# miloknowles/adaptive-stereo-icra-2021

Hardware: AMD Instinct MI355X
Metric: stereo pairs/sec (fwd+adapt-step), KITTI 1242x375 D=192 (higher is better)
Workload: dtype f32; 1 GPU; KITTI-2015 1242x375, maxdisp 192, k=4 (Dc=12, 24x78 cost volume), forward + one online-adapt step (train-mode BN, monodepth loss, clip 1.0, Adam lr 5e-5); pairs_per_gpu=4, global_batch=4, parallelism=dp1 (per-replica BatchNorm statistics, one flat RCCL gradient all-reduce), kernels=all hand-written HIP (no MIOpen/rocBLAS on the path)

## Files before the change

adaptive-stereo-icra-2021_amd/adaptive_stereo/_native.py:

```python
import ctypes
import os

import torch

_HERE = os.path.dirname(os.path.abspath(__file__))
LIB_PATH = os.path.join(_HERE, "libadaptive_stereo_hip.so")
BUILD_HINT = "build it with: make -C %s" % os.path.join(os.path.dirname(_HERE), "csrc")

c_int, c_float, c_i64, c_vp = ctypes.c_int, ctypes.c_float, ctypes.c_int64, ctypes.c_void_p


class Pcl(ctypes.Structure):
  _fields_ = [(n, ctypes.c_int32) for n in ("B", "D", "H", "W", "pd", "ph", "pw")]

  def numel(self):
    return self.B * (self.D + 2 * self.pd) * (self.H + 2 * self.ph) * (self.W + 2 * self.pw) * 32

  def voxels(self):
    return self.B * self.D * self.H * self.W

  def key(self):
    return (self.B, self.D, self.H, self.W, self.pd, self.ph, self.pw)


# ... 54 lines not shown
  "as_conv32to1_bnsums_ok": (c_int, [_P(Pcl), _P(ConvShape)]),
  "as_conv32to1_bnsums_parts": (c_int, [_P(Pcl)]),
  "as_conv32to1_dgrad_bnsums": (c_int, [c_vp, _P(Pcl), _P(ConvShape), c_vp, c_vp, c_vp, c_vp, c_vp, c_vp, c_float, c_vp, c_vp]),
  "as_wgrad_defer": (c_int, [c_int]),
  "as_wgrad_defer_pending": (c_int, []),
  "as_wgrad_defer_flush": (c_int, [c_vp]),
  "as_conv32_act_ok": (c_int, [_P(Pcl), _P(Pcl), _P(ConvShape)]),
  "as_conv32_act_parts": (c_int, []),
  "as_conv32_act_fwd": (c_int, [c_vp, c_vp, c_vp, c_vp, c_vp, _P(Pcl), c_vp, c_vp, c_float, c_vp, _P(Pcl), _P(ConvShape), c_vp, c_vp,
                                c_vp, c_vp]),
  "as_conv32_wino_ok": (c_int, [_P(Pcl), _P(Pcl), _P(ConvShape)]),
  "as_conv32_wino_parts": (c_int, []),
  "as_conv32_wino_pack_weights": (c_int, [c_vp, c_vp, c_int, c_vp]),
  "as_conv32_wino_fwd": (c_int, [c_vp, c_vp, c_vp, c_vp, c_vp, _P(Pcl), c_vp, c_vp, c_float, c_vp, _P(Pcl), _P(ConvShape), c_vp, c_vp,
                                 c_vp, c_vp]),
  "as_conv32_wino_eval": (c_int, [c_vp, _P(Pcl), _P(ConvShape), c_vp, c_vp, c_vp, c_vp, c_float, c_int, c_vp, c_vp]),
  "as_conv32_wino_bwd_data": (c_int, [c_vp, c_vp, _P(Pcl), _P(ConvShape), c_vp, c_vp, c_vp, c_vp, c_vp, c_float, c_vp, c_vp, c_vp, c_vp,
                                      c_vp, c_vp, c_vp, c_vp]),
  "as_conv32_wino_bwd_filter": (c_int, [c_vp, c_vp, _P(Pcl), _P(ConvShape), c_vp, c_vp, c_int, c_vp, c_vp]),
  "as_conv32_wino_bwd_parts": (c_int, []),
  "as_conv32_wino_bwd_workspace": (c_i64, []),
  "as_conv32_wino_bwd_generation": (c_int, [c_int]),
  "as_conv32_wino_bwd": (c_int, [c_vp, _P(Pcl), c_vp, c_vp, _P(Pcl), _P(ConvShape), c_vp, c_vp, c_vp, c_vp, c_vp, c_float, c_vp,
                                 c_vp, c_vp, c_vp, c_vp, c_vp, c_vp, c_vp, c_int, c_vp, c_vp, c_vp]),
  "as_conv32_wino_bwd_fused_parts": (c_int, []),
  "as_conv32_wino_bwd_fused_workspace": (c_i64, []),
  "as_conv32_wino_bwd_fused": (c_int, [c_vp, _P(Pcl), c_vp, c_vp, _P(Pcl), _P(ConvShape), c_vp, c_vp, c_vp, c_vp, c_vp, c_float, c_vp,
                                       c_vp, c_vp, c_vp, c_vp, c_vp, c_vp, c_int, c_vp, c_vp, c_vp]),
  "as_conv3d_wgrad_lds_assignment": (c_int, [c_int, c_int, c_int, c_vp, c_vp, c_vp]),
  "as_conv32_s2_enable": (c_int, [c_int]),
  "as_conv4_s2_enable": (c_int, [c_int]),
  "as_refine_out_ok": (c_int, [_P(Pcl)]),
  "as_refine_out_fwd": (c_int, [c_vp, c_vp, c_vp, c_vp, c_float, c_vp, _P(Pcl), c_vp, c_vp, c_vp, c_int, c_vp, c_vp]),
  "as_conv32_bwd_fused_ok": (c_int, [_P(Pcl), _P(Pcl), _P(ConvShape)]),
  "as_conv32_bwd_fused_parts": (c_int, []),
  "as_conv32_bwd_fused_workspace": (c_i64, []),
  "as_conv32_bwd_fused": (c_int, [c_vp, _P(Pcl), c_vp, c_vp, _P(Pcl), _P(ConvShape), c_vp, c_vp, c_vp, c_vp, c_vp, c_float, c_vp, c_vp,
                                  c_vp, c_vp, c_vp, c_vp, c_vp, c_int, c_vp, c_vp, c_vp]),
  "as_conv32_bnbwd_parts": (c_int, [_P(Pcl), _P(Pcl), _P(ConvShape)]),
  "as_conv32_fwd_bnbwd": (c_int, [c_vp, _P(Pcl), c_vp, c_vp, _P(Pcl), _P(ConvShape), c_vp, c_vp, c_vp, c_vp, c_vp, c_float,
                                  c_vp, c_vp]),
  "as_agg3d_ok": (c_int, [_P(Pcl)]),
  "as_agg3d_parts": (c_int, [_P(Pcl)]),
  "as_agg3d_fwd": (c_int, [c_vp, _P(Pcl), c_vp, c_vp, c_vp, c_vp, _P(BnMerge), c_vp, c_vp, c_int, c_vp, c_vp, c_float, c_vp, c_vp,
                           c_vp, c_vp]),
  "as_trunk_parts": (c_int, [_P(Pcl), c_int]),
  "as_trunk_fwd": (c_int, [c_vp, c_vp, _P(TrunkBn), c_vp, _P(Pcl), c_int, c_vp, c_vp, c_float, c_vp, c_vp, c_vp, c_vp, c_vp]),
  "as_trunk_finish_fwd": (c_int, [c_vp, _P(Pcl), c_vp, c_vp, c_int, c_int, _P(c_vp), _P(c_vp), c_float, c_vp]),
  "as_trunk_begin_bwd": (c_int, [c_vp, c_vp, c_int, _P(Pcl), c_vp, c_vp]),
  "as_trunk_bwd_workspace": (c_i64, [_P(Pcl), c_int]),
  "as_trunk_bwd": (c_int, [c_vp, c_vp, c_vp, c_vp, c_int, c_vp, c_vp, c_vp, c_vp, c_vp, c_vp, c_vp, c_vp, _P(Pcl), c_int, c_float,
                           c_vp, c_vp, c_int, c_vp, c_vp]),
  "as_trunk_finish_bwd": (c_int, [c_vp, c_int, c_int, _P(c_vp), _P(c_vp), c_int, c_vp]),
  "as_agg_tail_ok": (c_int, [_P(Pcl)]),
  "as_agg_tail_fwd": (c_int, [c_vp, _P(Pcl), c_vp, c_vp, _P(BnMerge), c_vp, c_vp, c_vp, c_float, c_vp, c_vp, c_vp, c_vp, c_vp]),
  "as_conv3d_out_fwd": (c_int, [c_vp, _P(Pcl), c_vp, c_vp, c_vp, c_vp]),
  "as_conv3d_out_bwd_workspace": (c_i64, [_P(Pcl)]),
  "as_conv3d_out_bwd": (c_int, [c_vp, c_vp, _P(Pcl), c_vp, c_vp, c_vp, c_vp, c_int, c_vp, c_vp]),
  "as_conv32to1_fwd": (c_int, [c_vp, _P(Pcl), _P(ConvShape), c_vp, c_vp, c_vp, c_int, c_vp, c_vp]),
  "as_conv32to1_bwd_workspace": (c_i64, [_P(Pcl), _P(ConvShape)]),
  "as_conv32to1_bwd": (c_int, [c_vp, c_vp, _P(Pcl), _P(ConvShape), c_vp, c_vp, c_vp, c_vp, c_int, c_vp, c_vp]),
  "as_pcl4_numel": (c_i64, [_P(Pcl)]),
  "as_pack_in4": (c_int, [c_vp, c_vp, c_int, c_vp, _P(Pcl), c_vp]),
  "as_conv4_pack_weights": (c_int, [c_vp, c_int, c_vp, _P(ConvShape), c_vp]),
  "as_conv4_wgrad_bnapply_ok": (c_int, [_P(Pcl), _P(Pcl), _P(ConvShape)]),
  "as_conv4_wgrad_bnapply_proj": (c_int, [c_vp, _P(Pcl), c_vp, c_vp, _P(Pcl), _P(ConvShape), c_int, c_vp, c_vp, c_vp, c_vp, c_float,
# ... 112 lines not shown
```

adaptive-stereo-icra-2021_amd/adaptive_stereo/hip_ops.py:

```python
import os
import torch

from . import _native as nat
from ._native import Pcl, ConvShape, call, ptr, stream, f32c

LEAKY_SLOPE = 0.2
BN_EPS = 1e-5
BN_MOMENTUM = 0.1

CONV3D_333 = ConvShape(3, 3, 3, 1, 1, 1, 1, 1)

_DIRECT_GRADS = True


def set_direct_grad_accumulation(flag: bool):
  global _DIRECT_GRADS
  _DIRECT_GRADS = bool(flag)


def grad_sinks(params):
  if not (_DIRECT_GRADS and torch.is_grad_enabled()):
    return None
  out = []
  for p in params:
# ... 107 lines not shown
  if not _DeferredReduce.on:
    return
  lib = nat.load()
  lib.as_wgrad_defer(0)
  _DeferredReduce.on = False
  call("as_wgrad_defer_flush", stream())
  _DeferredReduce.keep = []


_TAIL_BNSUMS = True
_HEAD_PROJ = True
_FWD_ACT = True
_WINOGRAD = os.environ.get("AS_DIAG_DIRECT_FORM") != "1"


def set_tail_bnsums(enabled):
  global _TAIL_BNSUMS
  prev, _TAIL_BNSUMS = _TAIL_BNSUMS, bool(enabled)
  return prev


def set_head_proj(enabled):
  global _HEAD_PROJ
  prev, _HEAD_PROJ = _HEAD_PROJ, bool(enabled)
  return prev


_REFINE_OUT = True


def set_refine_out(enabled):
  global _REFINE_OUT
  prev, _REFINE_OUT = _REFINE_OUT, bool(enabled)
  return prev


def set_head_staged(enabled):
  lib = nat.load()
  prev = lib.as_conv32_s2_enable(2) == 1 and lib.as_conv4_s2_enable(2) == 1
  lib.as_conv32_s2_enable(1 if enabled else 0)
  lib.as_conv4_s2_enable(1 if enabled else 0)
  return prev


def set_fwd_act(enabled):
  global _FWD_ACT
  prev, _FWD_ACT = _FWD_ACT, bool(enabled)
  return prev


_WINOGRAD_BWD = True
_WINOGRAD_BWD_ONE_LAUNCH = True


def set_winograd_bwd_one_launch(flag: bool):
  global _WINOGRAD_BWD_ONE_LAUNCH
  prev, _WINOGRAD_BWD_ONE_LAUNCH = _WINOGRAD_BWD_ONE_LAUNCH, bool(flag)
  return prev


def set_winograd(enabled, backward=None):
  global _WINOGRAD, _WINOGRAD_BWD
  prev, _WINOGRAD = _WINOGRAD, bool(enabled)
  _WINOGRAD_BWD = bool(enabled if backward is None else backward)
  return prev

# ... 1098 lines not shown
        a0 = POOL.get(g, dev)
        call("as_conv4_fwd", ptr(in4), g4, ptr(wp4), ptr(b0), ptr(a0), g, s33, 1, ptr(st0.scale), ptr(st0.shift),
             LEAKY_SLOPE, None, None, None, stream())
    if not need_bwd and z0 is not None:
      POOL.put(z0, g); z0 = None

    xs, zs, sts = [a0], [], []
    tail_fused = None
    if fused_act:
      xs = []
      z_prev, st_prev = z0, st0
      for l, dil in enumerate(REFINE_DILATIONS):
        wl, bl, gamma, beta = params[4 + 4 * l:8 + 4 * l]
        rm, rv = bn_buffers[1 + l]
        a_prev, z, st = block_forward_act(z_prev, xs[-1] if xs else None, st_prev, g, conv_shape_2d(dil), wl, bl, gamma, beta,
                                          rm, rv)
        xs.append(a_prev); zs.append(z); sts.append(st)
        z_prev, st_prev = z, st
      if _REFINE_OUT and lib.as_refine_out_ok(g) == 1:
        tail_fused = (z_prev, xs[-1], st_prev)
      else:
        xs.append(bn_act(z_prev, st_prev, g, residual=xs[-1]))
    else:
      for l, dil in enumerate(REFINE_DILATIONS):
        wl, bl, gamma, beta = params[4 + 4 * l:8 + 4 * l]
        rm, rv = bn_buffers[1 + l]
        z, a, st = block_forward(xs[-1], g, conv_shape_2d(dil), wl, bl, gamma, beta, rm, rv, train, True, need_bwd)
        zs.append(z); sts.append(st); xs.append(a)
        if not need_bwd:
          POOL.put(xs[-2], g)

    w_out, b_out = params[28], params[29]
    out = torch.empty(B, 1, H, W, dtype=torch.float32, device=dev)
    if tail_fused is not None:
      z6, a5, st6 = tail_fused
      a6 = POOL.get(g, dev)
      call("as_refine_out_fwd", ptr(z6), ptr(a5), ptr(st6.scale), ptr(st6.shift), LEAKY_SLOPE, ptr(a6), g, ptr(w_out), ptr(b_out),
           ptr(up), 1, ptr(out), stream())
      xs.append(a6)
    elif _REFINE_OUT and lib.as_refine_out_ok(g) == 1:
      call("as_refine_out_fwd", ptr(xs[-1]), None, None, None, LEAKY_SLOPE, None, g, ptr(w_out), ptr(b_out), ptr(up), 1, ptr(out),
           stream())
    else:
      call("as_conv32to1_fwd", ptr(xs[-1]), g, s33, ptr(w_out), ptr(b_out), ptr(up), 1, ptr(out), stream())

    if need_bwd:
      ctx.g, ctx.g4, ctx.train = g, g4, bool(train)
      ctx.sinks = sinks
      ctx.dims = (B, h, w, H, W, float(gain))
      ctx.in4, ctx.z0, ctx.st0 = in4, z0, st0
      ctx.xs, ctx.zs, ctx.sts = xs, zs, sts
      ctx.save_for_backward(out, *params)
    else:
      POOL.put(xs[-1], g); POOL.put(in4, g4, channels=4)
    return out

  @staticmethod
  def backward(ctx, g_out):
    out, *params = ctx.saved_tensors
    g, g4 = ctx.g, ctx.g4
    B, h, w, H, W, gain = ctx.dims
    dev = out.device
    lib = nat.load()
    s33 = conv_shape_2d(1)
    xs, zs, sts = ctx.xs, ctx.zs, ctx.sts
    grads = [None] * 30

    g_out = f32c(g_out)
    g_pre = torch.empty_like(out)
    call("as_relu_bwd", ptr(g_out), ptr(out), out.numel(), ptr(g_pre), stream())
    w_out = params[28]
    sinks = ctx.sinks
    g_a = POOL.get(g, dev)
    ws = _empty(lib.as_conv32to1_bwd_workspace(g, s33), dev)
    sums = None
    if _sink(sinks, 28) is not None and _sink(sinks, 29) is not None:
      if _TAIL_BNSUMS and ctx.train and _BN_SYNC is None and lib.as_conv32to1_bnsums_ok(g, s33) == 1:
        nws = _empty(lib.as_bn_bwd_workspace(g), dev)
        ev = fork_beside(lambda: call("as_conv32to1_bwd", ptr(g_pre), ptr(xs[6]), g, s33, ptr(w_out), None, ptr(sinks[28]),
                                      ptr(sinks[29]), 1, ptr(ws), stream()))
        call("as_conv32to1_dgrad_bnsums", ptr(g_pre), g, s33, ptr(w_out), ptr(g_a), ptr(zs[5]), ptr(sts[5].scale),
             ptr(sts[5].shift), ptr(sts[5].mean), LEAKY_SLOPE, ptr(nws), stream())
        join_beside(ev)
        sums = BnBwdSums(nws, lib.as_conv32to1_bnsums_parts(g))
      else:
        call("as_conv32to1_bwd", ptr(g_pre), ptr(xs[6]), g, s33, ptr(w_out), ptr(g_a), ptr(sinks[28]), ptr(sinks[29]), 1,
             ptr(ws), stream())
    else:
      g_wout, g_bout = torch.empty_like(w_out), _empty(1, dev)
      call("as_conv32to1_bwd", ptr(g_pre), ptr(xs[6]), g, s33, ptr(w_out), ptr(g_a), ptr(g_wout), ptr(g_bout), 0,
           ptr(ws), stream())
      grads[28], grads[29] = g_wout, g_bout

    for l in range(5, -1, -1):
      wl, bl, gamma, beta = params[4 + 4 * l:8 + 4 * l]
      next_bn = (zs[l - 1], sts[l - 1]) if l > 0 else (ctx.z0, ctx.st0)
      g_x, dW, db, g_gamma, g_beta, sums = block_backward(g_a, xs[l], zs[l], sts[l], wl, gamma, g,
                                                          conv_shape_2d(REFINE_DILATIONS[l]), ctx.train, True, True,
                                                          sinks[4 + 4 * l:8 + 4 * l] if sinks is not None else None,
                                                          sums, next_bn)
      grads[4 + 4 * l:8 + 4 * l] = [dW, db, g_gamma, g_beta]
      POOL.put(g_a, g); POOL.put(zs[l], g); POOL.put(xs[l + 1], g)
      g_a = g_x

    w0, b0, gamma0, beta0 = params[0:4]
    ws4 = _empty(lib.as_conv4_wgrad_workspace(g, s33), dev)
    all_sinks = all(_sink(sinks, i) is not None for i in range(4))
    if all_sinks and lib.as_conv4_wgrad_bnapply_ok(g4, g, s33) == 1:
      bws = sums.workspace if sums is not None else _empty(lib.as_bn_bwd_workspace(g), dev)
      st0 = ctx.st0
      bn_bwd_coefs(g_a, ctx.z0, st0, gamma0, g, ctx.train, sinks[2], sinks[3], True, bws, sums)
      coef = bws[lib.as_bn_bwd_coef_offset():]
      if _HEAD_PROJ and ctx.needs_input_grad[0] and not ctx.needs_input_grad[1]:
        w_proj = pack_special(w0, PACK_MIRROR_TAP, 9, 288,
                              lambda w_, o_: call("as_mirror_taps_ch0", ptr(w_), 4, ptr(o_), None, stream()))
        h_proj = _empty(B * 9 * H * W, dev)
        call("as_conv4_wgrad_bnapply_proj", ptr(ctx.in4), g4, ptr(g_a), ptr(ctx.z0), g, s33, 4, ptr(st0.scale), ptr(st0.shift),
             ptr(st0.mean), ptr(coef), LEAKY_SLOPE, ptr(w_proj), ptr(h_proj), ptr(sinks[0]), ptr(sinks[1]), 1, ptr(ws4),
             stream())
        g_z0 = None
      else:
        h_proj = None
        g_z0 = POOL.get(g, dev)
        call("as_conv4_wgrad_bnapply", ptr(ctx.in4), g4, ptr(g_a), ptr(ctx.z0), g, s33, 4, ptr(st0.scale), ptr(st0.shift),
             ptr(st0.mean), ptr(coef), LEAKY_SLOPE, ptr(g_z0), ptr(sinks[0]), ptr(sinks[1]), 1, ptr(ws4), stream())
      dW0 = db0 = g_gamma0 = g_beta0 = None
    else:
      h_proj = None
      g_z0, g_gamma0, g_beta0 = bn_act_bwd(g_a, ctx.z0, ctx.st0, gamma0, g, ctx.train, _sink(sinks, 2), _sink(sinks, 3), sums)
      if _sink(sinks, 0) is not None and _sink(sinks, 1) is not None:
        call("as_conv4_wgrad", ptr(ctx.in4), g4, ptr(g_z0), g, s33, 4, ptr(sinks[0]), ptr(sinks[1]), 1, ptr(ws4), stream())
        dW0 = db0 = None
      else:
        dW0 = torch.empty_like(w0); db0 = _empty(32, dev)
        call("as_conv4_wgrad", ptr(ctx.in4), g4, ptr(g_z0), g, s33, 4, ptr(dW0), ptr(db0), 0, ptr(ws4), stream())
# ... 219 lines not shown
```

adaptive-stereo-icra-2021_amd/csrc/refine_out.hip:

```cpp
#include "as_common.h"

#define RO_COLS 126
#ifndef RO_ROWS_ACT
#define RO_ROWS_ACT 32
#endif
#ifndef RO_ROWS_PLAIN
#define RO_ROWS_PLAIN 12
#endif
#define RO_PW 132

struct RefineOutArgs {
  const float* x;
  const float* skip;
  const float* scale;
  const float* shift;
  float* a_out;
  const float* w;
  const float* bias;
  const float* add_src;
  float* out;
  PclDev g;
  int nseg, nstrips, relu;
  float slope;
};

template <bool ACT>
__global__ __launch_bounds__(256) void refine_out_kernel(RefineOutArgs p) {
  __shared__ __attribute__((aligned(16))) char xrow[128 * 128];
  __shared__ float P[3][9][RO_PW];
  const int t = threadIdx.x, lane = t & 63, wave = t >> 6;
  const int h = lane >> 5, li = lane & 31;
  const int H = p.g.H, W = p.g.W;
  int blk = blockIdx.x;
  const int seg = blk % p.nseg; blk /= p.nseg;
  const int strip = blk % p.nstrips;
  const int b = blk / p.nstrips;
  const int x0 = seg * RO_COLS;
  constexpr int ROWS = ACT ? RO_ROWS_ACT : RO_ROWS_PLAIN;
  const int ya = strip * ROWS, yb = min(H, ya + ROWS);

  float Bw[16];
#pragma unroll
  for (int i = 0; i < 16; ++i) Bw[i] = li < 9 ? p.w[(16 * h + i) * 9 + li] : 0.f;
  const float bias = p.bias ? p.bias[0] : 0.f;

  const int cq = t & 7, v0 = t >> 3;
  const int lds_w = v0 * 128 + ((cq ^ ((v0 >> 1) & 7)) << 4);
  f32x4 sc = {0.f, 0.f, 0.f, 0.f}, sh = {0.f, 0.f, 0.f, 0.f};
  if (ACT) { sc = *reinterpret_cast<const f32x4*>(p.scale + cq * 4); sh = *reinterpret_cast<const f32x4*>(p.shift + cq * 4); }
  unsigned colmask = 0u, ownmask = 0u;
#pragma unroll
  for (int k = 0; k < 4; ++k) {
    const int v = v0 + 32 * k, xx = x0 - 1 + v;
    colmask |= ((xx >= 0 && xx < W) ? 1u : 0u) << k;
    ownmask |= ((v >= 1 && v <= RO_COLS && xx < W) ? 1u : 0u) << k;
  }
  const long row0 = (((long)b * p.g.Hp + p.g.ph) * p.g.Wp + (x0 - 1 + p.g.pw)) * 32 + t * 4;
  auto fetch = [&](int yi, f32x4 (&rz)[4], f32x4 (&rs)[4]) {
    const long off = row0 + (long)min(max(yi, 0), H - 1) * p.g.Wp * 32;
#pragma unroll
    for (int k = 0; k < 4; ++k) {
      rz[k] = *reinterpret_cast<const f32x4*>(p.x + off + k * 1024);
      if (ACT && p.skip) rs[k] = *reinterpret_cast<const f32x4*>(p.skip + off + k * 1024);
    }
  };
  const int mv = 32 * wave + li;
  const char* a_rd = xrow + mv * 128;
  const int a_sw = (mv >> 1) & 7;

  f32x4 rz[4], rs[4];
#pragma unroll
  for (int k = 0; k < 4; ++k) rs[k] = (f32x4){0.f, 0.f, 0.f, 0.f};
  fetch(ya - 1, rz, rs);
  for (int yi = ya - 1; yi <= yb; ++yi) {
    const bool row_in = yi >= 0 && yi < H;
    const bool row_own = yi >= ya && yi < yb;
#pragma unroll
    for (int k = 0; k < 4; ++k) {
      f32x4 y = rz[k];
      if (ACT) {
        y = y * sc + sh;
        y.x = y.x > 0.f ? y.x : y.x * p.slope; y.y = y.y > 0.f ? y.y : y.y * p.slope;
        y.z = y.z > 0.f ? y.z : y.z * p.slope; y.w = y.w > 0.f ? y.w : y.w * p.slope;
        if (p.skip) y += rs[k];
      }
      if (!row_in || !((colmask >> k) & 1u)) y = (f32x4){0.f, 0.f, 0.f, 0.f};
      *reinterpret_cast<f32x4*>(xrow + lds_w + k * 4096) = y;
      if (ACT && row_own && ((ownmask >> k) & 1u))
        *reinterpret_cast<f32x4*>(p.a_out + row0 + (long)yi * p.g.Wp * 32 + k * 1024) = y;
    }
    if (yi < yb) fetch(yi + 1, rz, rs);
    __syncthreads();
    f32x16 acc;
    {
      f32x4 xa[4];
#pragma unroll
      for (int q = 0; q < 4; ++q) xa[q] = *reinterpret_cast<const f32x4*>(a_rd + (((4 * h + q) ^ a_sw) << 4));
      const f32x16 zero = {0.f, 0.f, 0.f, 0.f, 0.f, 0.f, 0.f, 0.f, 0.f, 0.f, 0.f, 0.f, 0.f, 0.f, 0.f, 0.f};
      acc = __builtin_amdgcn_mfma_f32_32x32x2f32(xa[0].x, Bw[0], zero, 0, 0, 0);
      acc = __builtin_amdgcn_mfma_f32_32x32x2f32(xa[0].y, Bw[1], acc, 0, 0, 0);
      acc = __builtin_amdgcn_mfma_f32_32x32x2f32(xa[0].z, Bw[2], acc, 0, 0, 0);
      acc = __builtin_amdgcn_mfma_f32_32x32x2f32(xa[0].w, Bw[3], acc, 0, 0, 0);
#pragma unroll
      for (int q = 1; q < 4; ++q) {
        acc = __builtin_amdgcn_mfma_f32_32x32x2f32(xa[q].x, Bw[4 * q + 0], acc, 0, 0, 0);
        acc = __builtin_amdgcn_mfma_f32_32x32x2f32(xa[q].y, Bw[4 * q + 1], acc, 0, 0, 0);
        acc = __builtin_amdgcn_mfma_f32_32x32x2f32(xa[q].z, Bw[4 * q + 2], acc, 0, 0, 0);
        acc = __builtin_amdgcn_mfma_f32_32x32x2f32(xa[q].w, Bw[4 * q + 3], acc, 0, 0, 0);
      }
    }
    if (li < 9) {
      float* pr = &P[(yi + 1) % 3][li][32 * wave + 4 * h];
#pragma unroll
      for (int r = 0; r < 16; ++r) pr[(r & 3) + 8 * (r >> 2)] = acc[r];
    }
    __syncthreads();
    const int yo = yi - 1;
    if (yo >= ya && t < RO_COLS && x0 + t < W) {
      float s = bias;
#pragma unroll
      for (int ky = 0; ky < 3; ++ky) {
        const float (*pr)[RO_PW] = P[(yo + ky) % 3];
#pragma unroll
        for (int kx = 0; kx < 3; ++kx) s += pr[ky * 3 + kx][t + kx];
      }
      const long o = ((long)b * H + yo) * W + x0 + t;
      if (p.add_src) s += p.add_src[o];
      if (p.relu) s = s > 0.f ? s : 0.f;
      p.out[o] = s;
    }
  }
}

extern "C" int as_refine_out_ok(const as_pcl* g) {
  if (!as_pcl_ok(g)) return 0;
  return g->D == 1 && g->pd == 0 && g->ph >= 1 && g->pw >= 1 && (long)g->ph * (g->W + 2 * g->pw) >= 128 ? 1 : 0;
}

extern "C" int as_refine_out_fwd(const float* x, const float* skip, const float* scale, const float* shift, float slope,
                                 float* a_out, const as_pcl* g, const float* w, const float* bias, const float* add_src,
                                 int relu, float* out, void* stream) {
  AS_CHECK_ARG(as_refine_out_ok(g) == 1, "as_refine_out_fwd: geometry not supported (as_refine_out_ok() == 0)");
  AS_CHECK_ARG(x && w && out, "as_refine_out_fwd: null pointer");
  AS_CHECK_ARG((scale == nullptr) == (shift == nullptr) && (scale == nullptr) == (a_out == nullptr),
               "as_refine_out_fwd: scale, shift and a_out come together (the fused BatchNorm + LeakyReLU) or not at all");
  AS_CHECK_ARG(scale != nullptr || skip == nullptr, "as_refine_out_fwd: a skip connection needs the fused activation");
  AS_CHECK_ARG(a_out == nullptr || (a_out != x && a_out != skip), "as_refine_out_fwd: a_out must not alias an input");
  AS_CHECK_ARG(scale == nullptr || (slope > 0.f && slope < 1.f), "as_refine_out_fwd: slope must lie in (0, 1)");
  RefineOutArgs a;
  a.x = x; a.skip = skip; a.scale = scale; a.shift = shift; a.a_out = a_out; a.w = w; a.bias = bias; a.add_src = add_src;
  a.out = out; a.g = as_make_dev(g); a.relu = relu; a.slope = slope;
  a.nseg = as_div_up(g->W, RO_COLS); a.nstrips = as_div_up(g->H, scale ? RO_ROWS_ACT : RO_ROWS_PLAIN);
  const int grid = g->B * a.nseg * a.nstrips;
  if (scale) hipLaunchKernelGGL(refine_out_kernel<true>, dim3(grid), dim3(256), 0, (hipStream_t)stream, a);
  else hipLaunchKernelGGL(refine_out_kernel<false>, dim3(grid), dim3(256), 0, (hipStream_t)stream, a);
  AS_CHECK_LAUNCH("as_refine_out_fwd");
  return AS_OK;
}
```

adaptive-stereo-icra-2021_amd/csrc/softargmax.hip:

```cpp
#include "as_common.h"

struct OutGeom {
  int kd, kh, kw, pad_d, pad_h, pad_w, dil, ntaps;
  int tap_off[27];
};

struct OutConvArgs {
  const float* a;
  const float* w;
  const float* bias;
  const float* add_src;
  float* out;
  int relu;
  PclDev g;
  long M;
  OutGeom k;
};

__global__ __launch_bounds__(256) void conv32to1_fwd_kernel(OutConvArgs p) {
  __shared__ float sw[27 * 32];
  const int NT = p.k.ntaps;
  for (int i = threadIdx.x; i < NT * 32; i += 256) {
    const int t = i >> 5, c = i & 31;
    sw[i] = p.w[c * NT + t];
// ... 349 lines not shown
        const int vx = f >> 3;
        const f32x4 av = it == 0 ? a4[0][k4] : a4[1][k4];
        if (c4 == 0) gsum += sgc[1][vx + 1];
#pragma unroll
        for (int ky = 0; ky < 3; ++ky)
#pragma unroll
          for (int kx = 0; kx < 3; ++kx) acc[ky * 3 + kx] += sgc[2 - ky][vx + 2 - kx] * av;
      }
    }
  }
  float* out = p.partial + (long)blockIdx.x * (9 * 32 + 1);
#pragma unroll
  for (int tp = 0; tp < 9; ++tp) {
    __syncthreads();
    red[vl][c4 * 4 + 0] = acc[tp].x; red[vl][c4 * 4 + 1] = acc[tp].y;
    red[vl][c4 * 4 + 2] = acc[tp].z; red[vl][c4 * 4 + 3] = acc[tp].w;
    __syncthreads();
    if (threadIdx.x < 32) {
      float s = 0.f;
      for (int j = 0; j < 32; ++j) s += red[j][threadIdx.x];
      out[tp * 32 + threadIdx.x] = s;
    }
  }
  __syncthreads();
  if (c4 == 0) red[vl][0] = gsum;
  __syncthreads();
  if (threadIdx.x == 0) {
    float s = 0.f;
    for (int j = 0; j < 32; ++j) s += red[j][0];
    out[9 * 32] = s;
  }
}

static bool thin2d_applicable(const as_pcl* g, const as_conv_shape* s) {
  return g->D == 1 && s->kd == 1 && s->kh == 3 && s->kw == 3 && s->dil == 1 && s->stride == 1 && s->pad_h == 1 &&
         s->pad_w == 1 && g->ph >= 1 && g->pw >= 1 && (long)g->B * g->H * ((g->W + 127) / 128) < (1L << 31);
}

__global__ __launch_bounds__(256) void softargmax_fwd_kernel(const float* __restrict__ logits, int B, int D, long HW,
                                                              float* __restrict__ pred, int32_t* __restrict__ argmax,
                                                              float* __restrict__ fcs) {
  const long i = (long)blockIdx.x * 256 + threadIdx.x;
  if (i >= (long)B * HW) return;
  const long b = i / HW, pix = i % HW;
  const float* l = logits + b * D * HW + pix;
  float m1 = -INFINITY, m2 = -INFINITY, sum = 0.f;
  int am = 0;
  for (int d = 0; d < D; ++d) {
    const float v = l[d * HW];
    sum += v;
    if (v > m1) { m2 = m1; m1 = v; am = d; }
    else if (v > m2) { m2 = v; }
  }
  float se = 0.f;
  for (int d = 0; d < D; ++d) se += expf(l[d * HW] - m1);
  float acc = 0.f;
  for (int d = 0; d < D; ++d) acc += (expf(l[d * HW] - m1) / se) * (float)d;
  pred[i] = acc;
  if (argmax) argmax[i] = am;
  if (fcs) fcs[i] = (D > 2) ? m1 - (sum - m1 - m2) / (float)(D - 2) : 0.f;
}

__global__ __launch_bounds__(256) void softargmax_bwd_kernel(const float* __restrict__ logits, const float* __restrict__ g_pred,
                                                              const float* __restrict__ g_in, int B, int D, long HW,
                                                              float* __restrict__ g_logits) {
  const long i = (long)blockIdx.x * 256 + threadIdx.x;
// ... 116 lines not shown
    hipLaunchKernelGGL(conv32to1_wgrad_reduce_kernel, dim3(as_div_up(p.k.ntaps * 32 + 1, 4)), dim3(256), 0, st,
                       workspace, (int)nb, p.k.ntaps, g_w, g_bias, accumulate);
    AS_CHECK_LAUNCH("as_conv32to1_bwd(reduce)");
  }
  return AS_OK;
}

#define THIN_BNSUMS_BLOCKS 1024
extern "C" int as_conv32to1_bnsums_ok(const as_pcl* g, const as_conv_shape* s) {
  if (!g || !s || !as_pcl_ok(g)) return AS_ERR_ARG;
  return thin2d_applicable(g, s) ? 1 : 0;
}
extern "C" int as_conv32to1_bnsums_parts(const as_pcl* g) {
  if (!g || !as_pcl_ok(g)) return AS_ERR_ARG;
  const long nch = (long)g->B * g->H * ((g->W + 127) / 128);
  return (int)(nch < THIN_BNSUMS_BLOCKS ? nch : THIN_BNSUMS_BLOCKS);
}
extern "C" int as_conv32to1_dgrad_bnsums(const float* g_out, const as_pcl* g, const as_conv_shape* s, const float* w, float* g_a,
                                         const float* bn_z, const float* bn_scale, const float* bn_shift, const float* bn_mean,
                                         float slope, float* bn_workspace, void* stream) {
  AS_CHECK_ARG(g && s && as_pcl_ok(g) && thin2d_applicable(g, s), "as_conv32to1_dgrad_bnsums: configuration not supported");
  AS_CHECK_ARG(g_out && w && g_a && bn_z && bn_scale && bn_shift && bn_mean && bn_workspace, "as_conv32to1_dgrad_bnsums: null pointer");
  AS_CHECK_ARG(((uintptr_t)bn_workspace & 7) == 0, "as_conv32to1_dgrad_bnsums: workspace must be 8-byte aligned");
  Thin2dBwdArgs q;
  q.g_out = g_out; q.a = nullptr; q.w = w; q.g_a = g_a; q.partial = nullptr; q.g = as_make_dev(g);
  q.chunks_per_row = (g->W + 127) / 128; q.nchunks = g->B * g->H * q.chunks_per_row;
  q.bn_z = bn_z; q.bn_scale = bn_scale; q.bn_shift = bn_shift; q.bn_mean = bn_mean; q.slope = slope;
  q.bn_partial = reinterpret_cast<double*>(bn_workspace);
  hipLaunchKernelGGL(conv32to1_2d_dgrad_kernel<true>, dim3(as_conv32to1_bnsums_parts(g)), dim3(256), 0, (hipStream_t)stream, q);
  AS_CHECK_LAUNCH("as_conv32to1_dgrad_bnsums");
  return AS_OK;
}

static const as_conv_shape k333 = {3, 3, 3, 1, 1, 1, 1, 1};

extern "C" int as_conv3d_out_fwd(const float* a, const as_pcl* g, const float* w, const float* bias,
                                 float* logits, void* stream) {
  as_prof_mark(AS_PROF_OUTCONV_FWD, (hipStream_t)stream, 1, 0.0);
  const int e = as_conv32to1_fwd(a, g, &k333, w, bias, nullptr, 0, logits, stream);
  if (e == AS_OK && g) as_prof_mark(AS_PROF_OUTCONV_FWD, (hipStream_t)stream, 0, (128.0 + 4.0) * (double)g->B * g->D * g->H * g->W);
  return e;
}

extern "C" int64_t as_conv3d_out_bwd_workspace(const as_pcl* g) { return as_conv32to1_bwd_workspace(g, &k333); }

extern "C" int as_conv3d_out_bwd(const float* g_logits, const float* a, const as_pcl* g, const float* w,
                                 float* g_a, float* g_w, float* g_bias, int accumulate, float* workspace, void* stream) {
  AS_CHECK_ARG(g_a && g_w, "as_conv3d_out_bwd: null pointer");
  as_prof_mark(AS_PROF_OUTCONV_BWD, (hipStream_t)stream, 1, 0.0);
  const int e = as_conv32to1_bwd(g_logits, a, g, &k333, w, g_a, g_w, g_bias, accumulate, workspace, stream);
  if (e == AS_OK && g) as_prof_mark(AS_PROF_OUTCONV_BWD, (hipStream_t)stream, 0, (2 * 128.0 + 2 * 4.0) * (double)g->B * g->D * g->H * g->W);
  return e;
}

extern "C" int as_softargmax_fwd(const float* logits, int B, int D, int H, int W,
                                 float* pred, int32_t* argmax, float* fcs, void* stream) {
  AS_CHECK_ARG(logits && pred, "as_softargmax_fwd: null pointer");
  AS_CHECK_ARG(B > 0 && D > 0 && H > 0 && W > 0, "as_softargmax_fwd: bad shape");
  const long n = (long)B * H * W;
  as_prof_mark(AS_PROF_SOFTARGMAX_FWD, (hipStream_t)stream, 1, 0.0);
  hipLaunchKernelGGL(softargmax_fwd_kernel, dim3(as_div_up(n, 256)), dim3(256), 0, (hipStream_t)stream,
                     logits, B, D, (long)H * W, pred, argmax, fcs);
  as_prof_mark(AS_PROF_SOFTARGMAX_FWD, (hipStream_t)stream, 0, 4.0 * (double)n * (D + 3));
  AS_CHECK_LAUNCH("as_softargmax_fwd");
  return AS_OK;
}
// ... 14 lines not shown
```

include/adaptive_stereo_hip.h:

```cpp
#ifndef ADAPTIVE_STEREO_HIP_H_
#define ADAPTIVE_STEREO_HIP_H_

#include <stdint.h>

#ifdef __cplusplus
extern "C" {
#endif

#define AS_CHANNELS 32
#define AS_MAX_TAPS 32

typedef struct as_pcl {
  int32_t B, D, H, W;
  int32_t pd, ph, pw;
} as_pcl;

typedef struct as_conv_shape {
  int32_t kd, kh, kw;
  int32_t pad_d, pad_h, pad_w;
  int32_t dil;
  int32_t stride;
} as_conv_shape;

const char* as_last_error(void);
// ... 57 lines not shown
                        const float* scale, const float* shift, float slope, int residual, float* out, void* stream);

int as_conv32_wino_bwd_parts(void);
int64_t as_conv32_wino_bwd_workspace(void);
int as_conv32_wino_bwd_generation(int generation);
int as_conv32_wino_bwd_data(const float* g_a, const float* z, const as_pcl* g, const as_conv_shape* s,
                            const float* wino_wt, const float* scale, const float* shift, const float* mean,
                            const float* coef, float slope, const float* next_z, const float* next_scale,
                            const float* next_shift, const float* next_mean, float* g_z, float* g_x,
                            float* next_bn_workspace, void* stream);
int as_conv32_wino_bwd_filter(const float* x, const float* g_z, const as_pcl* g, const as_conv_shape* s, float* dW,
                              float* db, int accumulate, float* workspace, void* stream);
int as_conv32_wino_bwd(const float* x, const as_pcl* gin, const float* g_a, const float* z, const as_pcl* gout,
                       const as_conv_shape* s, const float* wino_wt, const float* scale, const float* shift,
                       const float* mean, const float* coef, float slope, const float* next_z,
                       const float* next_scale, const float* next_shift, const float* next_mean, float* g_z,
                       float* g_x, float* dW, float* db, int accumulate, float* next_bn_workspace,
                       float* workspace, void* stream);
int as_conv32_wino_bwd_fused_parts(void);
int64_t as_conv32_wino_bwd_fused_workspace(void);
int as_conv32_wino_bwd_fused(const float* x, const as_pcl* gin, const float* g_a, const float* z, const as_pcl* gout,
                             const as_conv_shape* s, const float* wino_wt, const float* scale, const float* shift,
                             const float* mean, const float* coef, float slope, const float* next_z,
                             const float* next_scale, const float* next_shift, const float* next_mean, float* g_x,
                             float* dW, float* db, int accumulate, float* next_bn_workspace, float* workspace, void* stream);

int as_conv32_s2_enable(int on);
int as_conv4_s2_enable(int on);

int as_refine_out_ok(const as_pcl* g);
int as_refine_out_fwd(const float* x, const float* skip, const float* scale, const float* shift, float slope, float* a_out,
                      const as_pcl* g, const float* w, const float* bias, const float* add_src, int relu, float* out,
                      void* stream);

typedef struct as_bn_merge {
  const float* stat_mean;
  const float* stat_m2;
  const float* stat_cnt;
  const float* gamma;
  const float* beta;
  float* running_mean;
  float* running_var;
  float* save_mean;
  float* save_invstd;
  float* scale;
  float* shift;
  int32_t nparts;
  float momentum;
  float eps;
} as_bn_merge;
int as_agg3d_ok(const as_pcl* g);
int as_agg3d_parts(const as_pcl* g);
int as_agg3d_fwd(const float* x, const as_pcl* g, const float* packed_w, const float* bias,
                 const float* in_scale, const float* in_shift, const as_bn_merge* in_bn, float* a_out,
                 float* z, int epilogue, const float* ep_scale, const float* ep_shift, float slope,
                 float* stat_mean, float* stat_m2, float* stat_cnt, void* stream);

int as_agg_tail_ok(const as_pcl* g);
int as_agg_tail_fwd(const float* x, const as_pcl* g, const float* in_scale, const float* in_shift,
                    const as_bn_merge* in_bn, float* a_out,
                    const float* w, const float* bias, float slope, float* logits, float* pred,
                    int32_t* argmax, float* fcs, void* stream);

typedef struct as_trunk_bn {
  const float* stat_mean;
  const float* stat_m2;
// ... 205 lines not shown
```

Before: 602.9 stereo pairs/s.

## Recompute refine tail activation in fused output-conv backward instead of storing it

The forward refine-output kernel no longer writes the last BN+LeakyReLU+skip activation when training without sync BN. A new backward kernel recomputes that activation from z and the skip tensor. In the same pass it folds in the ReLU gradient of the output, the 3x3 32-to-1 data and weight gradients, and the BN backward partial sums. This removes a full-resolution 32-channel store plus reload and a separate relu_bwd launch. In exchange the backward pass does extra reads of z and skip and some recompute.

```diff
diff --git a/adaptive-stereo-icra-2021_amd/adaptive_stereo/_native.py b/adaptive-stereo-icra-2021_amd/adaptive_stereo/_native.py
--- a/adaptive-stereo-icra-2021_amd/adaptive_stereo/_native.py
+++ b/adaptive-stereo-icra-2021_amd/adaptive_stereo/_native.py
@@ -110,6 +110,9 @@
   "as_conv4_s2_enable": (c_int, [c_int]),
   "as_refine_out_ok": (c_int, [_P(Pcl)]),
   "as_refine_out_fwd": (c_int, [c_vp, c_vp, c_vp, c_vp, c_float, c_vp, _P(Pcl), c_vp, c_vp, c_vp, c_int, c_vp, c_vp]),
+  "as_refine_out_bwd_workspace": (c_i64, [_P(Pcl)]),
+  "as_refine_out_bwd": (c_int, [c_vp, c_vp, c_vp, c_vp, c_vp, c_vp, c_vp, c_float, _P(Pcl), c_vp, c_vp, c_vp, c_vp, c_int, c_vp, c_vp,
+                                c_vp]),
   "as_conv32_bwd_fused_ok": (c_int, [_P(Pcl), _P(Pcl), _P(ConvShape)]),
   "as_conv32_bwd_fused_parts": (c_int, []),
   "as_conv32_bwd_fused_workspace": (c_i64, []),
diff --git a/adaptive-stereo-icra-2021_amd/adaptive_stereo/hip_ops.py b/adaptive-stereo-icra-2021_amd/adaptive_stereo/hip_ops.py
--- a/adaptive-stereo-icra-2021_amd/adaptive_stereo/hip_ops.py
+++ b/adaptive-stereo-icra-2021_amd/adaptive_stereo/hip_ops.py
@@ -163,6 +163,15 @@
 def set_refine_out(enabled):
   global _REFINE_OUT
   prev, _REFINE_OUT = _REFINE_OUT, bool(enabled)
+  return prev
+
+
+_OUT_BWD_FUSED = True
+
+
+def set_out_bwd_fused(enabled):
+  global _OUT_BWD_FUSED
+  prev, _OUT_BWD_FUSED = _OUT_BWD_FUSED, bool(enabled)
   return prev
 
 
@@ -1327,12 +1336,15 @@
 
     w_out, b_out = params[28], params[29]
     out = torch.empty(B, 1, H, W, dtype=torch.float32, device=dev)
+    a6_kept = True
     if tail_fused is not None:
       z6, a5, st6 = tail_fused
-      a6 = POOL.get(g, dev)
+      a6_kept = not (_OUT_BWD_FUSED and train and _BN_SYNC is None and lib.as_conv32to1_bnsums_ok(g, s33) == 1)
+      a6 = POOL.get(g, dev) if a6_kept else None
       call("as_refine_out_fwd", ptr(z6), ptr(a5), ptr(st6.scale), ptr(st6.shift), LEAKY_SLOPE, ptr(a6), g, ptr(w_out), ptr(b_out),
            ptr(up), 1, ptr(out), stream())
-      xs.append(a6)
+      if a6_kept:
+        xs.append(a6)
     elif _REFINE_OUT and lib.as_refine_out_ok(g) == 1:
       call("as_refine_out_fwd", ptr(xs[-1]), None, None, None, LEAKY_SLOPE, None, g, ptr(w_out), ptr(b_out), ptr(up), 1, ptr(out),
            stream())
@@ -1345,6 +1357,7 @@
       ctx.dims = (B, h, w, H, W, float(gain))
       ctx.in4, ctx.z0, ctx.st0 = in4, z0, st0
       ctx.xs, ctx.zs, ctx.sts = xs, zs, sts
+      ctx.a6_kept = a6_kept
       ctx.save_for_backward(out, *params)
     else:
       POOL.put(xs[-1], g); POOL.put(in4, g4, channels=4)
@@ -1362,14 +1375,31 @@
     grads = [None] * 30
 
     g_out = f32c(g_out)
-    g_pre = torch.empty_like(out)
-    call("as_relu_bwd", ptr(g_out), ptr(out), out.numel(), ptr(g_pre), stream())
     w_out = params[28]
     sinks = ctx.sinks
     g_a = POOL.get(g, dev)
-    ws = _empty(lib.as_conv32to1_bwd_workspace(g, s33), dev)
     sums = None
-    if _sink(sinks, 28) is not None and _sink(sinks, 29) is not None:
+    g_pre = None
+    if ctx.a6_kept or ctx.needs_input_grad[0]:
+      g_pre = torch.empty_like(out)
+      call("as_relu_bwd", ptr(g_out), ptr(out), out.numel(), ptr(g_pre), stream())
+    if not ctx.a6_kept:
+      ws = _empty(lib.as_refine_out_bwd_workspace(g), dev)
+      nws = _empty(lib.as_bn_bwd_workspace(g), dev)
+      if _sink(sinks, 28) is not None and _sink(sinks, 29) is not None:
+        g_wout, g_bout, acc = sinks[28], sinks[29], 1
+      else:
+        g_wout, g_bout, acc = torch.empty_like(w_out), _empty(1, dev), 0
+        grads[28], grads[29] = g_wout, g_bout
+      if g_pre is not None:
+        src, relu_of = g_pre, None
+      else:
+        src, relu_of = g_out, out
+      call("as_refine_out_bwd", ptr(src), ptr(relu_of), ptr(zs[5]), ptr(xs[5]), ptr(sts[5].scale), ptr(sts[5].shift),
+           ptr(sts[5].mean), LEAKY_SLOPE, g, ptr(w_out), ptr(g_a), ptr(g_wout), ptr(g_bout), acc, ptr(ws), ptr(nws), stream())
+      sums = BnBwdSums(nws, lib.as_conv32to1_bnsums_parts(g))
+    elif _sink(sinks, 28) is not None and _sink(sinks, 29) is not None:
+      ws = _empty(lib.as_conv32to1_bwd_workspace(g, s33), dev)
       if _TAIL_BNSUMS and ctx.train and _BN_SYNC is None and lib.as_conv32to1_bnsums_ok(g, s33) == 1:
         nws = _empty(lib.as_bn_bwd_workspace(g), dev)
         ev = fork_beside(lambda: call("as_conv32to1_bwd", ptr(g_pre), ptr(xs[6]), g, s33, ptr(w_out), None, ptr(sinks[28]),
@@ -1382,6 +1412,7 @@
         call("as_conv32to1_bwd", ptr(g_pre), ptr(xs[6]), g, s33, ptr(w_out), ptr(g_a), ptr(sinks[28]), ptr(sinks[29]), 1,
              ptr(ws), stream())
     else:
+      ws = _empty(lib.as_conv32to1_bwd_workspace(g, s33), dev)
       g_wout, g_bout = torch.empty_like(w_out), _empty(1, dev)
       call("as_conv32to1_bwd", ptr(g_pre), ptr(xs[6]), g, s33, ptr(w_out), ptr(g_a), ptr(g_wout), ptr(g_bout), 0,
            ptr(ws), stream())
@@ -1395,7 +1426,9 @@
                                                           sinks[4 + 4 * l:8 + 4 * l] if sinks is not None else None,
                                                           sums, next_bn)
       grads[4 + 4 * l:8 + 4 * l] = [dW, db, g_gamma, g_beta]
-      POOL.put(g_a, g); POOL.put(zs[l], g); POOL.put(xs[l + 1], g)
+      POOL.put(g_a, g); POOL.put(zs[l], g)
+      if l + 1 < len(xs):
+        POOL.put(xs[l + 1], g)
       g_a = g_x
 
     w0, b0, gamma0, beta0 = params[0:4]
diff --git a/adaptive-stereo-icra-2021_amd/csrc/refine_out.hip b/adaptive-stereo-icra-2021_amd/csrc/refine_out.hip
--- a/adaptive-stereo-icra-2021_amd/csrc/refine_out.hip
+++ b/adaptive-stereo-icra-2021_amd/csrc/refine_out.hip
@@ -24,7 +24,7 @@
   float slope;
 };
 
-template <bool ACT>
+template <bool ACT, bool STORE>
 __global__ __launch_bounds__(256) void refine_out_kernel(RefineOutArgs p) {
   __shared__ __attribute__((aligned(16))) char xrow[128 * 128];
   __shared__ float P[3][9][RO_PW];
@@ -86,7 +86,7 @@
       }
       if (!row_in || !((colmask >> k) & 1u)) y = (f32x4){0.f, 0.f, 0.f, 0.f};
       *reinterpret_cast<f32x4*>(xrow + lds_w + k * 4096) = y;
-      if (ACT && row_own && ((ownmask >> k) & 1u))
+      if (ACT && STORE && row_own && ((ownmask >> k) & 1u))
         *reinterpret_cast<f32x4*>(p.a_out + row0 + (long)yi * p.g.Wp * 32 + k * 1024) = y;
     }
     if (yi < yb) fetch(yi + 1, rz, rs);
@@ -142,8 +142,8 @@
                                  int relu, float* out, void* stream) {
   AS_CHECK_ARG(as_refine_out_ok(g) == 1, "as_refine_out_fwd: geometry not supported (as_refine_out_ok() == 0)");
   AS_CHECK_ARG(x && w && out, "as_refine_out_fwd: null pointer");
-  AS_CHECK_ARG((scale == nullptr) == (shift == nullptr) && (scale == nullptr) == (a_out == nullptr),
-               "as_refine_out_fwd: scale, shift and a_out come together (the fused BatchNorm + LeakyReLU) or not at all");
+  AS_CHECK_ARG((scale == nullptr) == (shift == nullptr) && (scale != nullptr || a_out == nullptr),
+               "as_refine_out_fwd: scale and shift come together (the fused BatchNorm + LeakyReLU); a_out only with them");
   AS_CHECK_ARG(scale != nullptr || skip == nullptr, "as_refine_out_fwd: a skip connection needs the fused activation");
   AS_CHECK_ARG(a_out == nullptr || (a_out != x && a_out != skip), "as_refine_out_fwd: a_out must not alias an input");
   AS_CHECK_ARG(scale == nullptr || (slope > 0.f && slope < 1.f), "as_refine_out_fwd: slope must lie in (0, 1)");
@@ -152,8 +152,9 @@
   a.out = out; a.g = as_make_dev(g); a.relu = relu; a.slope = slope;
   a.nseg = as_div_up(g->W, RO_COLS); a.nstrips = as_div_up(g->H, scale ? RO_ROWS_ACT : RO_ROWS_PLAIN);
   const int grid = g->B * a.nseg * a.nstrips;
-  if (scale) hipLaunchKernelGGL(refine_out_kernel<true>, dim3(grid), dim3(256), 0, (hipStream_t)stream, a);
-  else hipLaunchKernelGGL(refine_out_kernel<false>, dim3(grid), dim3(256), 0, (hipStream_t)stream, a);
+  if (scale && a_out) hipLaunchKernelGGL((refine_out_kernel<true, true>), dim3(grid), dim3(256), 0, (hipStream_t)stream, a);
+  else if (scale) hipLaunchKernelGGL((refine_out_kernel<true, false>), dim3(grid), dim3(256), 0, (hipStream_t)stream, a);
+  else hipLaunchKernelGGL((refine_out_kernel<false, false>), dim3(grid), dim3(256), 0, (hipStream_t)stream, a);
   AS_CHECK_LAUNCH("as_refine_out_fwd");
   return AS_OK;
 }
diff --git a/adaptive-stereo-icra-2021_amd/csrc/softargmax.hip b/adaptive-stereo-icra-2021_amd/csrc/softargmax.hip
--- a/adaptive-stereo-icra-2021_amd/csrc/softargmax.hip
+++ b/adaptive-stereo-icra-2021_amd/csrc/softargmax.hip
@@ -405,6 +405,156 @@
   }
 }
 
+struct RefineOutBwdArgs {
+  const float* g_out;
+  const float* out;
+  const float* z;
+  const float* skip;
+  const float* w;
+  const float* scale; const float* shift; const float* mean; float slope;
+  float* g_a;
+  float* partial;
+  double* bn_partial;
+  PclDev g;
+  int nchunks, chunks_per_row;
+};
+
+struct RefineOutBwdReq {
+  f32x4 z[4], s[4];
+  float g0, g1, o0, o1;
+};
+
+template <bool SKIP, bool RELU>
+__global__ __launch_bounds__(256) void refine_out_bwd_kernel(RefineOutBwdArgs p) {
+  __shared__ float sg[2][3][132];
+  __shared__ float red[2][32][33];
+  const int c4 = threadIdx.x & 7, vl = threadIdx.x >> 3;
+  f32x4 wv[9], acc_w[9];
+#pragma unroll
+  for (int k = 0; k < 9; ++k) {
+    wv[k] = (f32x4){p.w[(c4 * 4 + 0) * 9 + k], p.w[(c4 * 4 + 1) * 9 + k], p.w[(c4 * 4 + 2) * 9 + k], p.w[(c4 * 4 + 3) * 9 + k]};
+    acc_w[k] = (f32x4){0.f, 0.f, 0.f, 0.f};
+  }
+  const f32x4 bsc = *reinterpret_cast<const f32x4*>(p.scale + c4 * 4), bsh = *reinterpret_cast<const f32x4*>(p.shift + c4 * 4);
+  const f32x4 bmu = *reinterpret_cast<const f32x4*>(p.mean + c4 * 4);
+  f32x4 s_dy = {0.f, 0.f, 0.f, 0.f}, s_dx = {0.f, 0.f, 0.f, 0.f};
+  float gsum = 0.f;
+  const int i0 = threadIdx.x, i1 = threadIdx.x + 256;
+  const int r0 = i0 / 130, q0 = i0 - r0 * 130, r1 = i1 / 130, q1 = i1 - r1 * 130;
+  const int G = gridDim.x;
+
+  auto request = [&](int ch, RefineOutBwdReq& rq) {
+    const int rowi = ch / p.chunks_per_row, cx = ch - rowi * p.chunks_per_row;
+    const int y = rowi % p.g.H, b = rowi / p.g.H, x0 = cx * 128;
+    const int nf4 = min(128, p.g.W - x0) * 8;
+    const long voff = (((long)b * p.g.Hp + (y + p.g.ph)) * p.g.Wp + (x0 + p.g.pw)) * 32;
+#pragma unroll
+    for (int k4 = 0; k4 < 4; ++k4) {
+      const int f = min((int)threadIdx.x + 256 * k4, nf4 - 1);
+      rq.z[k4] = *reinterpret_cast<const f32x4*>(p.z + voff + f * 4);
+      if (SKIP) rq.s[k4] = *reinterpret_cast<const f32x4*>(p.skip + voff + f * 4);
+    }
+    const long a0 = ((long)b * p.g.H + min(max(y - 1 + r0, 0), p.g.H - 1)) * p.g.W + min(max(x0 - 1 + q0, 0), p.g.W - 1);
+    const long a1 = ((long)b * p.g.H + min(max(y - 1 + r1, 0), p.g.H - 1)) * p.g.W + min(max(x0 - 1 + q1, 0), p.g.W - 1);
+    rq.g0 = p.g_out[a0];
+    if (RELU) rq.o0 = p.out[a0];
+    if (i1 < 3 * 130) {
+      rq.g1 = p.g_out[a1];
+      if (RELU) rq.o1 = p.out[a1];
+    }
+  };
+
+  auto chunk = [&](int ch, const RefineOutBwdReq& cur, RefineOutBwdReq& nxt, float (*sgc)[132]) {
+    const int rowi = ch / p.chunks_per_row, cx = ch - rowi * p.chunks_per_row;
+    const int y = rowi % p.g.H, b = rowi / p.g.H, x0 = cx * 128;
+    const int nf4 = min(128, p.g.W - x0) * 8;
+    {
+      const int yy = y - 1 + r0, xx = x0 - 1 + q0;
+      float v = RELU ? (cur.o0 > 0.f ? cur.g0 : 0.f) : cur.g0;
+      sgc[r0][q0] = (yy >= 0 && yy < p.g.H && xx >= 0 && xx < p.g.W) ? v : 0.f;
+    }
+    if (i1 < 3 * 130) {
+      const int yy = y - 1 + r1, xx = x0 - 1 + q1;
+      float v = RELU ? (cur.o1 > 0.f ? cur.g1 : 0.f) : cur.g1;
+      sgc[r1][q1] = (yy >= 0 && yy < p.g.H && xx >= 0 && xx < p.g.W) ? v : 0.f;
+    }
+    __syncthreads();
+    if (ch + G < p.nchunks) request(ch + G, nxt);
+    float* dst = p.g_a + (((long)b * p.g.Hp + (y + p.g.ph)) * p.g.Wp + (x0 + p.g.pw)) * 32;
+#pragma unroll
+    for (int k4 = 0; k4 < 4; ++k4) {
+      const int f = threadIdx.x + 256 * k4;
+      if (f < nf4) {
+        const int vx = f >> 3;
+        const f32x4 zz = cur.z[k4];
+        const f32x4 yy = zz * bsc + bsh;
+        f32x4 a = yy;
+        a.x = a.x > 0.f ? a.x : a.x * p.slope; a.y = a.y > 0.f ? a.y : a.y * p.slope;
+        a.z = a.z > 0.f ? a.z : a.z * p.slope; a.w = a.w > 0.f ? a.w : a.w * p.slope;
+        if (SKIP) a += cur.s[k4];
+        if (c4 == 0) gsum += sgc[1][vx + 1];
+        f32x4 acc = {0.f, 0.f, 0.f, 0.f};
+#pragma unroll
+        for (int ky = 0; ky < 3; ++ky)
+#pragma unroll
+          for (int kx = 0; kx < 3; ++kx) {
+            const float gv = sgc[2 - ky][vx + 2 - kx];
+            acc += gv * wv[ky * 3 + kx];
+            acc_w[ky * 3 + kx] += gv * a;
+          }
+        *reinterpret_cast<f32x4*>(dst + f * 4) = acc;
+        f32x4 gy;
+        gy.x = yy.x > 0.f ? acc.x : acc.x * p.slope; gy.y = yy.y > 0.f ? acc.y : acc.y * p.slope;
+        gy.z = yy.z > 0.f ? acc.z : acc.z * p.slope; gy.w = yy.w > 0.f ? acc.w : acc.w * p.slope;
+        s_dy += gy; s_dx += gy * (zz - bmu);
+      }
+    }
+  };
+
+  RefineOutBwdReq ra, rb;
+  int ch = blockIdx.x;
+  if (ch < p.nchunks) request(ch, ra);
+  while (ch < p.nchunks) {
+    chunk(ch, ra, rb, sg[0]);
+    ch += G;
+    if (ch >= p.nchunks) break;
+    chunk(ch, rb, ra, sg[1]);
+    ch += G;
+  }
+
+  __syncthreads();
+  red[0][vl][c4 * 4 + 0] = s_dy.x; red[0][vl][c4 * 4 + 1] = s_dy.y; red[0][vl][c4 * 4 + 2] = s_dy.z; red[0][vl][c4 * 4 + 3] = s_dy.w;
+  red[1][vl][c4 * 4 + 0] = s_dx.x; red[1][vl][c4 * 4 + 1] = s_dx.y; red[1][vl][c4 * 4 + 2] = s_dx.z; red[1][vl][c4 * 4 + 3] = s_dx.w;
+  __syncthreads();
+  if (threadIdx.x < 64) {
+    const int which = threadIdx.x >> 5, c = threadIdx.x & 31;
+    double sum = 0.0;
+    for (int j = 0; j < 32; ++j) sum += (double)red[which][j][c];
+    p.bn_partial[(long)blockIdx.x * 64 + which * 32 + c] = sum;
+  }
+  float* out = p.partial + (long)blockIdx.x * (9 * 32 + 1);
+#pragma unroll
+  for (int tp = 0; tp < 9; ++tp) {
+    __syncthreads();
+    red[0][vl][c4 * 4 + 0] = acc_w[tp].x; red[0][vl][c4 * 4 + 1] = acc_w[tp].y;
+    red[0][vl][c4 * 4 + 2] = acc_w[tp].z; red[0][vl][c4 * 4 + 3] = acc_w[tp].w;
+    __syncthreads();
+    if (threadIdx.x < 32) {
+      float s = 0.f;
+      for (int j = 0; j < 32; ++j) s += red[0][j][threadIdx.x];
+      out[tp * 32 + threadIdx.x] = s;
+    }
+  }
+  __syncthreads();
+  if (c4 == 0) red[0][vl][0] = gsum;
+  __syncthreads();
+  if (threadIdx.x == 0) {
+    float s = 0.f;
+    for (int j = 0; j < 32; ++j) s += red[0][j][0];
+    out[9 * 32] = s;
+  }
+}
+
 static bool thin2d_applicable(const as_pcl* g, const as_conv_shape* s) {
   return g->D == 1 && s->kd == 1 && s->kh == 3 && s->kw == 3 && s->dil == 1 && s->stride == 1 && s->pad_h == 1 &&
          s->pad_w == 1 && g->ph >= 1 && g->pw >= 1 && (long)g->B * g->H * ((g->W + 127) / 128) < (1L << 31);
@@ -587,6 +737,38 @@
   return AS_OK;
 }
 
+static const as_conv_shape k133 = {1, 3, 3, 0, 1, 1, 1, 1};
+extern "C" int64_t as_refine_out_bwd_workspace(const as_pcl* g) {
+  if (!g || !as_pcl_ok(g)) return -1;
+  return (int64_t)THIN_BNSUMS_BLOCKS * (9 * 32 + 1);
+}
+extern "C" int as_refine_out_bwd(const float* g_out, const float* out, const float* z, const float* skip, const float* scale,
+                                 const float* shift, const float* mean, float slope, const as_pcl* g, const float* w, float* g_a,
+                                 float* g_w, float* g_bias, int accumulate, float* workspace, float* bn_workspace, void* stream) {
+  AS_CHECK_ARG(g && as_pcl_ok(g) && thin2d_applicable(g, &k133), "as_refine_out_bwd: geometry not supported (as_conv32to1_bnsums_ok() == 0)");
+  AS_CHECK_ARG(g_out && z && scale && shift && mean && w && g_a && workspace && bn_workspace, "as_refine_out_bwd: null pointer");
+  AS_CHECK_ARG(g_a != z && g_a != skip, "as_refine_out_bwd: g_a must not alias an input");
+  AS_CHECK_ARG(slope > 0.f && slope < 1.f, "as_refine_out_bwd: slope must lie in (0, 1)");
+  AS_CHECK_ARG(((uintptr_t)bn_workspace & 7) == 0, "as_refine_out_bwd: bn_workspace must be 8-byte aligned");
+  RefineOutBwdArgs q;
+  q.g_out = g_out; q.out = out; q.z = z; q.skip = skip; q.w = w; q.scale = scale; q.shift = shift; q.mean = mean; q.slope = slope;
+  q.g_a = g_a; q.partial = workspace; q.bn_partial = reinterpret_cast<double*>(bn_workspace); q.g = as_make_dev(g);
+  q.chunks_per_row = (g->W + 127) / 128; q.nchunks = g->B * g->H * q.chunks_per_row;
+  const int nb = as_conv32to1_bnsums_parts(g);
+  hipStream_t st = (hipStream_t)stream;
+  if (skip && out) hipLaunchKernelGGL((refine_out_bwd_kernel<true, true>), dim3(nb), dim3(256), 0, st, q);
+  else if (skip) hipLaunchKernelGGL((refine_out_bwd_kernel<true, false>), dim3(nb), dim3(256), 0, st, q);
+  else if (out) hipLaunchKernelGGL((refine_out_bwd_kernel<false, true>), dim3(nb), dim3(256), 0, st, q);
+  else hipLaunchKernelGGL((refine_out_bwd_kernel<false, false>), dim3(nb), dim3(256), 0, st, q);
+  AS_CHECK_LAUNCH("as_refine_out_bwd");
+  if (g_w || g_bias) {
+    hipLaunchKernelGGL(conv32to1_wgrad_reduce_kernel, dim3(as_div_up(9 * 32 + 1, 4)), dim3(256), 0, st, workspace, nb, 9, g_w, g_bias,
+                       accumulate);
+    AS_CHECK_LAUNCH("as_refine_out_bwd(reduce)");
+  }
+  return AS_OK;
+}
+
 static const as_conv_shape k333 = {3, 3, 3, 1, 1, 1, 1, 1};
 
 extern "C" int as_conv3d_out_fwd(const float* a, const as_pcl* g, const float* w, const float* bias,
diff --git a/include/adaptive_stereo_hip.h b/include/adaptive_stereo_hip.h
--- a/include/adaptive_stereo_hip.h
+++ b/include/adaptive_stereo_hip.h
@@ -113,6 +113,10 @@
 int as_refine_out_fwd(const float* x, const float* skip, const float* scale, const float* shift, float slope, float* a_out,
                       const as_pcl* g, const float* w, const float* bias, const float* add_src, int relu, float* out,
                       void* stream);
+int64_t as_refine_out_bwd_workspace(const as_pcl* g);
+int as_refine_out_bwd(const float* g_out, const float* out, const float* z, const float* skip, const float* scale,
+                      const float* shift, const float* mean, float slope, const as_pcl* g, const float* w, float* g_a,
+                      float* g_w, float* g_bias, int accumulate, float* workspace, float* bn_workspace, void* stream);
 
 typedef struct as_bn_merge {
   const float* stat_mean;
```

Result: no change. 598.5 stereo pairs/s (-0.7%).
